# zhang-tao-whu/DVIS_Plus

Hardware: AMD Instinct MI355X
Metric: frames/sec DVIS++ R50 offline, 720p T=30 synthetic (higher is better)
Workload: dtype f32 (storage, accumulation, results; the segmenter's dense layers - R50 convolutions from 128 channels on, pixel-decoder projections and FPN output convolution, the deformable encoder's projections and FFN, the decoder's key / value projections - multiply each fp32 operand as two f16 terms on the f1

## Files before the change

### dvis_plus_amd/backbone.py

```python
import torch
import torch.nn.functional as F
from torch import nn

from . import derived, functions as Fn
from .registry import BACKBONE_REGISTRY, ShapeSpec


class FrozenBatchNorm2d(nn.Module):
    def __init__(self, num_features, eps=1e-5):
        super().__init__()
        self.num_features, self.eps = num_features, eps
        self.register_buffer("weight", torch.ones(num_features))
        self.register_buffer("bias", torch.zeros(num_features))
        self.register_buffer("running_mean", torch.zeros(num_features))
        self.register_buffer("running_var", torch.ones(num_features) - eps)

    def scale_shift(self):
        scale = self.weight * (self.running_var + self.eps).rsqrt()
        return scale, self.bias - self.running_mean * scale

    def forward(self, x):
        scale, shift = self.scale_shift()
        return x * scale.reshape(1, -1, 1, 1) + shift.reshape(1, -1, 1, 1)

# ... 151 lines not shown
        return {k: ShapeSpec(channels=self._out_channels[k], stride=2 ** int(k[3:]))
                for k in self._out_features}

    @staticmethod
    def _chain_blocks(stage):
        blocks = []
        for b in stage:
            convs = [b.conv1, b.conv2, b.conv3] + ([b.shortcut] if b.shortcut is not None else [])
            if any(c.stride != (1, 1) or c.dilation != (1, 1) or c.groups != 1 for c in convs) or b.conv2.padding != (1, 1) \
                    or any(c.padding != (0, 0) for c in (b.conv1, b.conv3)):
                return None
            (w1, b1), (w2, b2), (w3, b3) = b.conv1.folded(), b.conv2.folded(), b.conv3.folded()
            ws, bs = b.shortcut.folded() if b.shortcut is not None else (None, None)
            if any(key_is_channels_last(w) for w in (w1, w2, w3) + ((ws,) if ws is not None else ())):
                return None
            blocks.append(dict(w1=w1, b1=b1, w2=w2, b2=b2, w3=w3, b3=b3, ws=ws, bs=bs))
        return blocks

    def _forward_live(self, x):
        out = {}
        x = F.max_pool2d(F.relu(self.stem.conv1.live(x)), kernel_size=3, stride=2, padding=1)
        for name in self.stage_names:
            for b in getattr(self, name):
                y = F.relu(b.conv2.live(F.relu(b.conv1.live(x))))
                x = F.relu(b.conv3.live(y) + (x if b.shortcut is None else b.shortcut.live(x)))
            if name in self._out_features:
                out[name] = x
        return out

    @Fn.fp32_island
    def forward(self, x):
        if torch.is_grad_enabled() and any(p.requires_grad for p in self.parameters()):
            return self._forward_live(Fn.f32(x))
        out = {}
        x = self.stem(Fn.f32(x))
        for name in self.stage_names:
            stage = getattr(self, name)
            blocks = self._chain_blocks(stage) if name == "res2" and x.is_cuda and not torch.is_grad_enabled() else None
            if blocks is not None and Fn.bneck_stage_x3_ok(x, blocks):
                x = Fn.bneck_stage_x3(x, blocks)
            else:
                x = stage(x)
            if name in self._out_features:
                out[name] = x
        return out


def build_resnet50():
    return ResNet((3, 4, 6, 3))


@BACKBONE_REGISTRY.register()
def build_resnet_backbone(cfg, input_shape=None):
    r = cfg.MODEL.get("RESNETS", {}) if hasattr(cfg.MODEL, "get") else getattr(cfg.MODEL, "RESNETS", {})
    get = (lambda k, d: r.get(k, d)) if hasattr(r, "get") else (lambda k, d: getattr(r, k, d))
    if int(get("DEPTH", 50)) != 50 or bool(get("STRIDE_IN_1X1", False)) or get("NORM", "FrozenBN") != "FrozenBN":
        raise NotImplementedError("dvis_plus_amd serves ResNet-50 with FrozenBN and STRIDE_IN_1X1 False "
                                  "(the reference's R50 configs); use detectron2's builder for other ResNets")
    return ResNet((3, 4, 6, 3), tuple(get("OUT_FEATURES", ["res2", "res3", "res4", "res5"])))
```

### dvis_plus_amd/functions.py

```python
import collections
import ctypes
import math
import os
import threading

import torch
from torch.autograd import Function
from torch.autograd.function import once_differentiable

from . import cpu_ops, derived, native
from .cpu_ops import ms_deform_attn_core_pytorch


def _torch_path(op, x, why):
    if os.environ.get("DVIS_STRICT", "1") != "0" and x.is_cuda and not torch.is_grad_enabled():
        raise RuntimeError(f"DVIS_STRICT: {op} would run its torch formulation on a GPU tensor ({why}; shape "
                           f"{tuple(x.shape)}, dtype {x.dtype}, contiguous {x.is_contiguous()})")


class no_autocast:

    def __enter__(self):
        import contextlib
        self._stack = contextlib.ExitStack()
# ... 2377 lines not shown
                native.dev_ptr(out, "out"), N, C, K, H, W, 1 if relu else 0, native.stream_ptr(x.device))
        native.check(rc, "dvis_conv3x3s2")
        return out
    y = torch.nn.functional.conv2d(x, weight, None, 2, 1)
    if bias is None and not relu:
        return y
    return bias_act_(y, None if bias is None else bias.detach(), None, relu)


def conv7x7s2_stem(x, weight, bias=None, relu=False, own=None):
    N, C, H, W = x.shape
    K = weight.shape[0]
    ok = x.is_cuda and x.dtype == torch.float32 and weight.dtype == torch.float32 and tuple(weight.shape) == (64, 3, 7, 7) \
        and not (torch.is_grad_enabled() and (x.requires_grad or weight.requires_grad)) \
        and bool(native.lib().dvis_conv7x7s2_supported(C, K, H, W))
    if own and not ok:
        raise RuntimeError(f"conv7x7s2_stem(own=True): C={C} K={K} H={H} W={W} is not served (dvis_conv7x7s2_supported)")
    if ok and (own or (own is None and WINOGRAD_DEFAULT and S2_DEFAULT)):
        uf = _fp32_pack(weight, "conv7x7s2", 10240, native.lib().dvis_conv7x7s2_pack, "dvis_conv7x7s2_pack")
        x = x if x.is_contiguous() else x.contiguous()
        out = torch.empty((N, 64, H // 2, W // 2), dtype=torch.float32, device=x.device)
        with torch.cuda.device(x.device):
            rc = native.lib().dvis_conv7x7s2(native.dev_ptr(x, "x"), native.dev_ptr(uf, "uf"),
                                             None if bias is None else native.dev_ptr(bias.detach(), "bias"),
                                             native.dev_ptr(out, "out"), N, H, W, 1 if relu else 0, native.stream_ptr(x.device))
        native.check(rc, "dvis_conv7x7s2")
        return out
    y = torch.nn.functional.conv2d(x, weight, None, 2, 3)
    if bias is None and not relu:
        return y
    return bias_act_(y, None if bias is None else bias.detach(), None, relu)


def conv3x3_bias_act(x, weight, bias=None, relu=False, winograd=None):
    if winograd is None and weight.shape[1] >= 128 and conv3x3_x3_ok(x, weight, 1):
        return conv3x3_x3(x, weight, bias, None, relu, 1)
    use = WINOGRAD_DEFAULT if winograd is None else winograd
    if use and x.is_cuda and x.dim() == 4 and x.dtype == torch.float32 and weight.dtype == torch.float32 \
            and tuple(weight.shape[2:]) == (3, 3) and not (torch.is_grad_enabled() and (x.requires_grad or weight.requires_grad)):
        N, C, H, W = x.shape
        K = weight.shape[0]
        served = weight.shape[1] == C and native.lib().dvis_conv3x3_winograd_supported(C, K, H, W)
        if winograd and not served:
            raise RuntimeError(f"conv3x3_bias_act(winograd=True): shape C={C} K={K} H={H} W={W} is not served "
                               "(dvis_conv3x3_winograd_supported)")
        if served:
            x = x if x.is_contiguous() else x.contiguous()
            uf = _winograd_weights(weight)
            out = torch.empty((N, K, H, W), dtype=torch.float32, device=x.device)
            with torch.cuda.device(x.device):
                rc = native.lib().dvis_conv3x3_winograd(
                    native.dev_ptr(x, "x"), native.dev_ptr(uf, "uf"),
                    None if bias is None else native.dev_ptr(bias.detach(), "bias"), native.dev_ptr(out, "out"), N, C, K, H, W,
                    1 if relu else 0, native.stream_ptr(x.device))
            native.check(rc, "dvis_conv3x3_winograd")
            return out
    y = torch.nn.functional.conv2d(x, weight, None, 1, 1)
    if bias is None and not relu:
        return y
    return bias_act_(y, None if bias is None else bias.detach(), None, relu)


def bias_act_(x, bias=None, res=None, relu=True):
    N, C, H, W = x.shape
    if not (x.is_cuda and x.dtype == torch.float32 and x.is_contiguous()
            and (res is None or (res.is_contiguous() and res.shape == x.shape and res.dtype == torch.float32))
# ... 700 lines not shown
```

### dvis_plus_amd/meta_architecture.py

```python
import os

import numpy as np
import torch
from torch import nn

from . import d2
from . import functions as Fn
from . import native
from . import postprocess as PP
from .clip_shard import ClipShard, EmulatedShard
from .d2 import configurable
from .registry import META_ARCH_REGISTRY, SEM_SEG_HEADS_REGISTRY


def _get(node, key, default):
    if hasattr(node, "get"):
        return node.get(key, default)
    return getattr(node, key, default)


@SEM_SEG_HEADS_REGISTRY.register()
class MaskFormerHead(nn.Module):

    @configurable
# ... 36 lines not shown

@SEM_SEG_HEADS_REGISTRY.register()
class FCCLIPHead(MaskFormerHead):

    @configurable
    def __init__(self, input_shape=None, *, num_classes, pixel_decoder, loss_weight=1.0, ignore_value=-1, transformer_predictor,
                 transformer_in_feature):
        super().__init__(input_shape, num_classes=num_classes, pixel_decoder=pixel_decoder, loss_weight=loss_weight,
                         ignore_value=ignore_value, transformer_predictor=transformer_predictor,
                         transformer_in_feature=transformer_in_feature)

    @classmethod
    def from_config(cls, cfg, input_shape):
        ret = MaskFormerHead.from_config.__func__(cls, cfg, input_shape)
        del ret["return_transformer_feature"]
        return ret

    @Fn.fp32_island
    def forward(self, features, mask=None):
        mask_features, _, multi_scale_features = self.pixel_decoder.forward_features(features)
        return self.predictor(multi_scale_features, mask_features, mask, text_classifier=features["text_classifier"],
                              num_templates=features["num_templates"])

    def layers(self, features, mask=None):
        return self.forward(features, mask)


def segmenter_frames_per_call(n, H, W, requested=0):
    chunk = min(requested or max(1, n), max(1, n))
    if 0 < chunk < n:
        calls = (n + chunk - 1) // chunk
        chunk = (n + calls - 1) // calls
    return max(1, chunk)


class _VideoBase(nn.Module):

    @configurable
    def __init__(self, *, backbone, sem_seg_head, num_queries, object_mask_threshold=0.8, overlap_threshold=0.8,
                 n_things=0, size_divisibility=32, pixel_mean=(123.675, 116.280, 103.530),
                 pixel_std=(58.395, 57.120, 57.375), tracker=None, refiner=None, task="vis", max_num=20,
                 window_size=3, segmenter_chunk=0, metadata=None, criterion=None,
                 sem_seg_postprocess_before_inference=True, num_frames=1, window_inference=True, max_iter_num=0,
                 use_cl=False, reference_outputs=False):
        super().__init__()
        self.backbone, self.sem_seg_head, self.tracker, self.refiner = backbone, sem_seg_head, tracker, refiner
        self.num_queries = num_queries
        self.object_mask_threshold, self.overlap_threshold = object_mask_threshold, overlap_threshold
        self.metadata = metadata
        ids = d2.thing_ids_from_metadata(metadata, video=True)
        self.thing_ids = frozenset(range(int(n_things))) if ids is None else ids
        self.num_frames, self.window_inference = num_frames, window_inference
        self.criterion, self.max_iter_num, self.use_cl, self.iter = criterion, max_iter_num, use_cl, 0
        self.size_divisibility = size_divisibility
        self.register_buffer("pixel_mean", torch.tensor(pixel_mean, dtype=torch.float32).view(-1, 1, 1), False)
        self.register_buffer("pixel_std", torch.tensor(pixel_std, dtype=torch.float32).view(-1, 1, 1), False)
        assert task in ("vis", "vss", "vps")
        self.task, self.max_num = task, max_num
        self.reference_outputs = bool(reference_outputs)
        self.window_size = window_size
        self.segmenter_chunk = segmenter_chunk
        self.keep = False
        self._clip_shard = None
        self.pipeline_rounds = int(os.environ.get("DVIS_PIPELINE_ROUNDS", "1"))
        self._tracker_stream = None
        self.owner_rounds = os.environ.get("DVIS_OWNER_ROUNDS", "1") != "0"
# ... 43 lines not shown
                                       noise_mode=_get(trk, "NOISE_MODE", "none"),
                                       noise_ratio=_get(trk, "NOISE_RATIO", 0.5), mask_dim=mf.HIDDEN_DIM,
                                       class_num=cfg.MODEL.SEM_SEG_HEAD.NUM_CLASSES), hidden

    @staticmethod
    def _new_tracker_stream():
        return torch.cuda.Stream()

    @property
    def clip_shard(self):
        if isinstance(self._clip_shard, EmulatedShard):
            return self._clip_shard
        world = torch.distributed.get_world_size() if torch.distributed.is_initialized() else 1
        if self._clip_shard is None or self._clip_shard.world != world:
            self._clip_shard = ClipShard()
        return self._clip_shard

    def preprocess(self, frames):
        x = frames if torch.is_tensor(frames) else torch.stack([f.to(self.device) for f in frames])
        H, W = x.shape[-2:]
        d = self.size_divisibility
        Hp, Wp = ((H + d - 1) // d * d, (W + d - 1) // d * d) if d > 1 else (H, W)
        x = x.to(self.device)
        if x.is_cuda and x.dim() == 4 and not torch.is_grad_enabled():
            exact = x.dtype in (torch.int8, torch.int16, torch.float16, torch.bfloat16, torch.bool)
            x = (x.to(torch.float32) if exact else x).contiguous()
        if Fn.normalize_pad_ok(x, self.pixel_mean):
            return Fn.normalize_pad(x, self.pixel_mean, self.pixel_std, Hp, Wp), (H, W)
        x = (x.to(torch.float32) - self.pixel_mean) / self.pixel_std
        if (Hp, Wp) != (H, W):
            x = torch.nn.functional.pad(x, (0, Wp - W, 0, Hp - H))
        return x, (H, W)

    def prepare_targets(self, batched_inputs, images):
        Hp, Wp = images.shape[-2:]
        out = []
        for video in batched_inputs:
            frames = video["instances"]
            masks = torch.zeros((len(frames[0].gt_ids), len(frames), Hp, Wp), dtype=torch.bool, device=self.device)
            ids, classes = [], []
            for f, inst in enumerate(frames):
                m = getattr(inst.gt_masks, "tensor", inst.gt_masks).to(self.device)
                masks[:, f, :m.shape[-2], :m.shape[-1]] = m.bool()
                ids.append(inst.gt_ids.to(self.device)[:, None])
                classes.append(inst.gt_classes.to(self.device)[:, None])
            ids = torch.cat(ids, dim=1)
            classes = torch.cat(classes, dim=1).max(dim=1)[0]
            valid = (ids != -1).any(dim=-1)
            out.append({"labels": classes[valid], "ids": ids[valid], "masks": masks[valid].float()})
        return out

    def encode(self, images):
        chunk = segmenter_frames_per_call(len(images), images.shape[-2], images.shape[-1], self.segmenter_chunk)
        ms, mf = [], []
        for s in range(0, len(images), chunk):
            with Fn.x3_stage("backbone"):
                feats = self.backbone(images[s:s + chunk])
            f, _, m = self.sem_seg_head.pixel_decoder.forward_features(feats)
            mf.append(f)
            ms.append(m)
        if len(mf) == 1:
            return ms[0], mf[0]
        return [torch.cat(level, 0) for level in zip(*ms)], torch.cat(mf, 0)

    def decode(self, multi_scale, mask_features):
        if len(mask_features) == 0:
            pred = self.sem_seg_head.predictor
            C2, Q = self.tracker.decoder_norm.weight.shape[0], self.num_queries
            z = lambda *shape: mask_features.new_zeros(shape)
            return z(0, Q, C2), z(0, Q, C2), z(0, Q, pred.class_embed.out_features)
        out = self.sem_seg_head.predictor(multi_scale, mask_features, None)
        return (out["pred_embds"][0].permute(1, 2, 0), out["pred_embds_without_norm"][0].permute(1, 2, 0),
                out["pred_logits"][0])

    def segment(self, images):
        ms, mf = self.encode(images)
        return (*self.decode(ms, mf), mf)

    def _segmenter_graph_ok(self, images):
        limit = int(os.environ.get("DVIS_SEGMENTER_GRAPH", "8"))
        ok = bool(images.is_cuda and 0 < len(images) <= limit and not torch.is_grad_enabled() and self.debug_stages is None
                  and getattr(self.sem_seg_head.predictor, "debug_masks", None) is None)
        if ok and self._seg_graph is None:
            from .graphs import GraphRunner
            self._seg_graph = GraphRunner(lambda im: tuple(self.segment(im)), max_entries=4)
        return ok

    def _guard_snapshot(self):
        return Fn.x3_range_snapshot(self.device) if not getattr(self, "_x3_off", False) else None

# ... 117 lines not shown

        def run():
            with self._x3_scope(), Fn.x3_stage("backbone"):
                features = self.backbone(images)
            self._guard_verify(self._guard_snapshot())
            return features

        def again():
            with torch.no_grad():
                for b, v in saved:
                    b.copy_(v)
            return run()
        try:
            return run()
        except Fn.X3RangeError as e:
            return self._x3_rerun(e, again)

    @staticmethod
    def frame_decoder_loss_reshape(outputs, targets):
        def one(d):
            return {"pred_masks": d["pred_masks"].permute(0, 2, 1, 3, 4).flatten(0, 1).unsqueeze(2),
                    "pred_logits": d["pred_logits"].flatten(0, 1)}
        out = {**outputs, **one(outputs)}
        if "aux_outputs" in outputs:
            out["aux_outputs"] = [one(a) for a in outputs["aux_outputs"]]
        return out, _VideoBase._per_frame_targets(targets)

    @Fn.fp32_island
    def _forward_eval(self, batched_inputs):
        assert len(batched_inputs) == 1
        from . import functions as Fn
        from .tracker import match_chain
        video = batched_inputs[0]
        images, img_size = self.preprocess(video["image"])
        pred = self.sem_seg_head.predictor
        with self._x3_scope():
            ms, mask_features = self.encode(images)
            dec, logits, _ = pred._final_heads(pred._run_layers(ms, mask_features), mask_features, False)
        try:
            self._guard_verify(self._guard_snapshot())
        except Fn.X3RangeError as e:
            return self._x3_rerun(e, lambda: self._forward_eval(batched_inputs))
        T, Q, _ = dec.shape
        idx = torch.arange(Q, device=dec.device).unsqueeze(0).repeat(T, 1)
        if T > 1:
            align = self._alignment_embeds(pred, dec)
            nrm = align / align.norm(dim=-1, keepdim=True)
            cost = 1 - torch.bmm(nrm[1:], nrm[:-1].transpose(1, 2))
            idx[1:] = torch.from_numpy(match_chain(cost)).to(dec.device)
        ar = torch.arange(T, device=dec.device)[:, None]
        cls = logits[ar, idx].mean(0)
        K = self.sem_seg_head.num_classes
        scores, labels, slot = PP.vis_select(cls, K, self.TOPK)
        emb = pred.mask_embed(dec[ar, idx[:, slot]])
        masks = Fn.mask_logits(emb.contiguous(), mask_features).permute(1, 0, 2, 3)
        out_hw = (video.get("height", img_size[0]), video.get("width", img_size[1]))
        masks = PP.resize2_gt0(masks, images.shape[-2:], img_size, out_hw)
        out = {"image_size": tuple(out_hw), "pred_scores": scores.tolist(), "pred_labels": labels.tolist(),
               "pred_masks": [m for m in masks], "pred_ids": slot.tolist(), "aligned_indices": idx}
        return PP.to_reference_format(out) if self.reference_outputs else out


@META_ARCH_REGISTRY.register()
class CTMinVIS(MinVIS):

    @configurable
    def __init__(self, *, image_matcher=None, cl_plugin=None, **kwargs):
# ... 205 lines not shown
                                                   self.classes_references_memory))
        return self._weighted(losses)

    @staticmethod
    def frame_decoder_loss_reshape(outputs, targets, image_outputs=None):
        def one(d):
            b, q, t, h, w = d["pred_masks"].shape
            return {"pred_masks": d["pred_masks"].reshape(b, q, 1, t * h, w), "pred_logits": d["pred_logits"][:, 0]}
        out = one(outputs)
        out["pred_embds"] = outputs["pred_embds"]
        out["aux_outputs"] = [one(a) for a in outputs.get("aux_outputs", ())]
        if image_outputs is not None:
            b, q, t, h, w = image_outputs["pred_masks"].shape
            image_outputs = {"pred_masks": image_outputs["pred_masks"].reshape(b, q, 1, t * h, w),
                             "pred_logits": image_outputs["pred_logits"].mean(dim=1)}
        flat = []
        for t_ in targets:
            g, t, h, w = t_["masks"].shape
            flat.append({**t_, "masks": t_["masks"].reshape(g, 1, t * h, w)})
        return image_outputs, out, flat

    @torch.no_grad()
    def _segment_phase(self, video, shift=0):
        return self._segment_round([video], shift)[0]

    @torch.no_grad()
    def _segment_round(self, videos, shift=0, rotate=True):
        metas, batches = [], []
        for j, video in enumerate(videos):
            frames = video["image"]
            T = len(frames)
            sh = shift + j if rotate else shift
            lo, hi = self.clip_shard.local_range(T, sh)
            images, img_size = self.preprocess(frames[lo:hi] if hi > lo else frames[:1])
            metas.append(dict(video=video, T=T, lo=lo, hi=hi, shift=sh, img_size=img_size,
                              padded=tuple(images.shape[-2:])))
            batches.append(images if hi > lo else images[:0])
        mask_dim = self.sem_seg_head.predictor.mask_embed.layers[-1].out_features
        merged = len(videos) > 1 and len({m["padded"] for m in metas}) == 1 and sum(len(b) for b in batches) > 0 \
            and (self.clip_shard.world > 1 or self.clip_shard.force or "DVIS_ROUND_CLIPS" in os.environ)

        def run(images):
            if len(images):
                return self.segment(images)
            mf = images.new_zeros((0, mask_dim, images.shape[-2] // 4, images.shape[-1] // 4))
            return (*self.decode(None, mf), mf)
        with self._x3_scope():
            if merged:
                outs = run(torch.cat(batches, 0))
                sizes = [len(b) for b in batches]
                parts = [o.split(sizes, 0) for o in outs]
                per_clip = [tuple(p[j] for p in parts) for j in range(len(videos))]
            else:
                per_clip = [run(b) for b in batches]
        guard = self._guard_snapshot()
        for m, (e, e_nn, lg, mf) in zip(metas, per_clip):
            m.update(embds=e, embds_nn=e_nn, logits=lg, mf=mf, guard=guard)
            if self.debug_stages is not None:
                self.debug_stages.update(mask_features=mf)
        return metas

    @property
    def _resume(self):
        return bool(self.keep) and not self.window_inference

    def _track_core(self, embds, embds_nn):
        to_bctq = lambda z: z.permute(2, 0, 1).unsqueeze(0)
        embds, embds_nn = embds.contiguous(), embds_nn.contiguous()
        track = self.tracker(to_bctq(embds), None, resume=self._resume, frame_embeds_no_norm=to_bctq(embds_nn),
                             need_masks=False)
        ref = self.refiner(track["pred_embds"], to_bctq(embds_nn), None, need_masks=False)
        cls, aux = PP.mean_logits(ref["pred_logits"], track["pred_logits"])
        if self.debug_stages is not None:
            self.debug_stages.update(frame_embds=to_bctq(embds), frame_embds_no_norm=to_bctq(embds_nn),
                                     instance_embds=track["pred_embds"], online_logits=track["pred_logits"],
                                     refiner_embds=ref["pred_embds"], refiner_logits=ref["pred_logits"],
                                     refiner_mask_embed=ref["mask_embed"])
        return ref["mask_embed"], cls, aux

    def _finish_phase(self, st, mask_embed, cls, aux):
        video, lo, hi = st["video"], st["lo"], st["hi"]
        emb_local = mask_embed[:, lo:hi]
# ... 165 lines not shown
        return self._forward_eval(batched_inputs)

    @torch.no_grad()
    @Fn.fp32_island
    def _forward_eval(self, batched_inputs):
        assert len(batched_inputs) == 1 and not self.training
        video = batched_inputs[0]
        if self.pipeline_rounds <= 1:
            try:
                out = self._track_phase(self._segment_phase(video))
            except Fn.X3RangeError as e:
                out = self._x3_rerun(e, lambda: self._track_phase(self._segment_phase(video)))
            return PP.to_reference_format(out) if self.reference_outputs else out
        self.keep = bool(video.get("keep", False))
        frames = video["image"]
        T = len(frames)
        shard = self.clip_shard
        plan, k = shard.round_plan(T, self.pipeline_rounds)
        to_bctq = lambda z: z.permute(2, 0, 1).unsqueeze(0)
        overlap = len(plan) > 1 and self.device.type == "cuda"
        main = torch.cuda.current_stream() if overlap else None
        if overlap and self._tracker_stream is None:
            self._tracker_stream = self._new_tracker_stream()

        local_ids = [i for (_, _, lo, hi) in plan for i in range(lo, hi)]
        contiguous = local_ids == list(range(local_ids[0], local_ids[0] + len(local_ids))) if local_ids else True
        if not local_ids:
            mine = frames[:0] if torch.is_tensor(frames) else []
        elif contiguous:
            mine = frames[local_ids[0]:local_ids[0] + len(local_ids)]
        else:
            mine = frames[torch.as_tensor(local_ids, device=frames.device)] if torch.is_tensor(frames) \
                else [frames[i] for i in local_ids]
        images, img_size = self.preprocess(mine if local_ids else frames[:1])
        if not local_ids:
            images = images[:0]
            pred = self.sem_seg_head.predictor
            multi_scale = None
            mask_features = images.new_zeros((0, pred.mask_embed.layers[-1].out_features, images.shape[-2] // 4,
                                              images.shape[-1] // 4))
        else:
            multi_scale, mask_features = self.encode(images)
        padded = images.shape[-2:]
        offsets, o = [], 0
        for (_, _, lo, hi) in plan:
            offsets.append((o, o + hi - lo))
            o += hi - lo

        def run_segmenter(c):
            start, end, lo, hi = plan[c]
            a, b = offsets[c]
            whole = a == 0 and b == len(local_ids)
            ms = None if multi_scale is None else (multi_scale if whole else _slice_maps(multi_scale, a, b))
            e, e_nn, lg = self.decode(ms, mask_features[a:b])
            (e, e_nn, lg), work = shard.all_gather_frames([e, e_nn, lg], end - start, per=k, async_op=True)
            done = torch.cuda.Event() if overlap else None
            if overlap:
                done.record(main)
            return dict(embds=e, embds_nn=e_nn, logits=lg, work=work, done=done)

        def run_tracker(c, seg):
            if seg["work"] is not None:
                seg["work"].wait()
            return self.tracker(to_bctq(seg["embds"]), None, resume=self._resume or c > 0,
                                frame_embeds_no_norm=to_bctq(seg["embds_nn"]), need_masks=False)

        segs, tracks = [run_segmenter(0)], []
# ... 282 lines not shown
```

### dvis_plus_amd/native.py

```python
import ctypes
import os

import torch

_HERE = os.path.dirname(os.path.abspath(__file__))
LIB_PATH = os.environ.get("DVIS_HIP_LIB") or os.path.join(_HERE, "lib", "libdvis_hip.so")

F32, F64, F16, BF16 = 0, 1, 2, 3
_DTYPE = {torch.float32: F32, torch.float64: F64, torch.float16: F16, torch.bfloat16: BF16}

_c = ctypes
_i, _i64, _p, _f = _c.c_int, _c.c_int64, _c.c_void_p, _c.c_float

SIGNATURES = {
    "dvis_last_error": (_c.c_char_p, []),
    "dvis_version": (_i, []),
    "dvis_msda_forward": (_i, [_i, _p, _p, _p, _p, _p, _i, _i, _i, _i, _i, _i, _i, _p, _p]),
    "dvis_msda_backward": (_i, [_i, _p, _p, _p, _p, _p, _p, _i, _i, _i, _i, _i, _i, _i, _p, _p, _p, _p]),
    "dvis_msda_backward_det_ws_bytes": (_i64, [_i, _i, _i, _i]),
    "dvis_msda_backward_det": (_i, [_p, _p, _p, _p, _p, _p, _i, _i, _i, _i, _i, _i, _i, _p, _p, _p, _p, _p]),
    "dvis_msda_fused_backward_ws_bytes": (_i64, [_i, _i, _i, _i]),
    "dvis_msda_fused_backward": (_i, [_p, _p, _p, _p, _i, _p, _i64, _p, _i64, _p, _i, _i, _i, _i, _i, _i, _i, _p, _p, _p, _p, _p]),
    "dvis_msda_fused_forward": (_i, [_p, _p, _p, _p, _i, _p, _i64, _p, _i64, _i, _i, _i, _i, _i, _i, _i, _p, _p, _p]),
    "dvis_msda_fused_forward_h": (_i, [_i, _p, _p, _p, _p, _i, _p, _i64, _p, _i64, _i, _i, _i, _i, _i, _i, _i, _p, _p, _p]),
    "dvis_nchw_to_tokens": (_i, [_p, _p, _i64, _i, _i64, _i64, _i64, _p]),
    "dvis_tokens_to_nchw": (_i, [_p, _p, _i64, _i, _i64, _i64, _i64, _p]),
    "dvis_normalize_pad": (_i, [_p, _i, _p, _i64, _i, _i, _i, _i, _i, _p, _p, _p]),
    "dvis_nchw_to_tokens_affine": (_i, [_p, _p, _p, _p, _p, _p, _i64, _i, _i64, _i64, _i64, _p]),
    "dvis_mask_logits": (_i, [_p, _p, _i, _i, _i, _i64, _p, _p]),
    "dvis_mask_logits_backward_ws_bytes": (_i64, [_i, _i, _i, _i64]),
    "dvis_mask_logits_backward": (_i, [_p, _p, _i, _i, _i, _i64, _p, _p, _p, _p]),
    "dvis_attn_mask": (_i, [_p, _p, _i, _i, _i, _i, _i, _i, _i, _p, _p, _p]),
    "dvis_center_pool3": (_i, [_p, _i64, _i, _i, _p, _p, _p, _p]),
    "dvis_attn_mask_pooled": (_i, [_p, _p, _i, _i, _i, _i, _i, _p, _p, _p]),
    "dvis_mask_gemm_plan": (_i, [_i, _i, _i, _i, _i, _i, _i, _i, _i, _i, _p, _i]),
    "dvis_attention_ws_bytes": (_i64, [_i, _i, _i, _i]),
    "dvis_attention_ws_bytes_k": (_i64, [_i, _i, _i, _i, _i]),
    "dvis_attention_plan": (_i, [_i, _i, _i, _i, _i, _i64, _i64, _i, _p]),
    "dvis_attention_forward": (_i, [_p, _p, _p, _p, _p, _p, _p, _p, _p, _p, _i, _i, _i, _i, _i, _f, _p, _p]),
    "dvis_attention_forward_k": (_i, [_p, _p, _p, _p, _p, _p, _p, _p, _p, _p, _i, _i, _i, _i, _i, _f, _p, _p, _i]),
    "dvis_attention_backward": (_i, [_p, _p, _p, _p, _p, _p, _p, _p, _p, _p, _p, _i, _i, _i, _i, _i, _f, _p]),
    "dvis_attention_backward_threads": (_i, [_i]),
    "dvis_masked_attention_backward_ws_bytes": (_i64, [_i, _i, _i, _i]),
    "dvis_masked_attention_backward": (_i, [_p, _p, _p, _p, _p, _p, _p, _p, _p, _p, _p, _p, _p, _i, _i, _i, _i, _i, _f, _p, _p]),
    "dvis_masked_attention_backward_plan": (_i, [_i, _i, _i, _p]),
    "dvis_add_layernorm": (_i, [_p, _p, _i64, _p, _p, _p, _i64, _i, _f, _p]),
    "dvis_add_layernorm_pos": (_i, [_p, _p, _i64, _p, _p, _p, _p, _i64, _p, _i64, _i, _f, _p]),
    "dvis_bias_act": (_i, [_p, _p, _p, _i64, _i, _i64, _i, _p]),
    "dvis_conv3x3_winograd_supported": (_i, [_i, _i, _i, _i]),
    "dvis_conv3x3_winograd_pack": (_i, [_p, _p, _i, _i, _p]),
    "dvis_conv3x3_winograd": (_i, [_p, _p, _p, _p, _i, _i, _i, _i, _i, _i, _p]),
    "dvis_conv3x3s2_supported": (_i, [_i, _i, _i, _i]),
    "dvis_conv3x3s2_pack": (_i, [_p, _p, _i, _i, _p]),
    "dvis_conv3x3s2": (_i, [_p, _p, _p, _p, _i, _i, _i, _i, _i, _i, _p]),
    "dvis_conv7x7s2_supported": (_i, [_i, _i, _i, _i]),
    "dvis_conv7x7s2_pack": (_i, [_p, _p, _p]),
    "dvis_conv7x7s2": (_i, [_p, _p, _p, _p, _i, _i, _i, _i, _p]),
    "dvis_conv1x1_mfma_supported": (_i, [_i, _i, _i64]),
    "dvis_conv1x1_mfma_pack": (_i, [_p, _p, _i, _i, _p]),
    "dvis_conv1x1_mfma": (_i, [_p, _p, _p, _p, _p, _i, _i, _i, _i64, _i, _p]),
    "dvis_conv1x1s2_mfma": (_i, [_p, _p, _p, _p, _p, _i, _i, _i, _i, _i, _i, _p]),
    "dvis_conv1x1_supported": (_i, [_i, _i, _i64]),
    "dvis_conv1x1_bias_act": (_i, [_p, _p, _p, _p, _p, _i, _i, _i, _i64, _i, _p]),
    "dvis_bias_relu_maxpool": (_i, [_p, _p, _p, _i64, _i, _i, _i, _p]),
    "dvis_group_norm_affine": (_i, [_p, _p, _p, _p, _p, _i64, _i, _i, _i64, _f, _p]),
    "dvis_scale_shift_act": (_i, [_p, _p, _p, _i64, _i64, _i, _p]),
    "dvis_group_norm_finalize": (_i, [_p, _p, _p, _p, _p, _i64, _i, _i, _i64, _f, _p]),
    "dvis_upsample_add_affine": (_i, [_p, _p, _p, _p, _p, _i64, _i, _i, _i, _i, _p]),
    "dvis_upsample_add": (_i, [_p, _p, _p, _i64, _i, _i, _i, _i, _p]),
    "dvis_dwconv3x3_tokens": (_i, [_p, _p, _i64, _i, _i, _i, _i, _p, _p, _i, _p]),
    "dvis_dwconv3x3_tokens_backward_ws_bytes": (_i64, [_i, _i, _i, _i]),
    "dvis_dwconv3x3_tokens_backward": (_i, [_p, _p, _p, _p, _i, _i64, _i, _i, _i, _i, _p, _p, _p, _p, _p]),
    "dvis_adapter_res2": (_i, [_p, _p, _p, _p, _p, _p, _i, _i, _i, _i, _p]),
    "dvis_vps_argmax": (_i, [_p, _i64, _i64, _p, _i, _i, _i, _i, _i, _i, _i, _i, _i, _i, _p, _p, _p, _p]),
    "dvis_vss_argmax": (_i, [_p, _i64, _i64, _p, _i, _i, _i, _i, _i, _i, _i, _i, _i, _i, _i, _i, _p, _p]),
    "dvis_resize2_gt0": (_i, [_p, _i64, _i64, _i, _i, _i, _i, _i, _i, _i, _i, _i, _i, _p, _p]),
    "dvis_resize2": (_i, [_p, _i64, _i64, _i, _i, _i, _i, _i, _i, _i, _i, _i, _i, _i, _p, _p]),
    "dvis_lsap_solve": (_i, [_p, _i, _i, _p]),
    "dvis_match_chain": (_i, [_p, _i, _i, _p]),
    "dvis_gemm_nt": (_i, [_p, _i64, _i64, _p, _i64, _i64, _p, _p, _i64, _i64, _p, _i64, _i64, _i, _i, _i, _i, _i, _i, _p]),
    "dvis_gemm_nt_bb": (_i, [_p, _i64, _i64, _p, _i64, _i64, _p, _i64, _p, _i64, _i64, _p, _i64, _i64, _i, _i, _i, _i, _i, _i,
                             _p]),
    "dvis_gemm_ln": (_i, [_p, _i64, _p, _i64, _p, _p, _f, _p, _p, _f, _p, _i64, _p, _i64, _p, _p, _i64, _p, _i64, _i, _i, _i,
                          _i, _i, _p]),
    "dvis_gemm_ln_supported": (_i, [_i, _i, _i, _i]),
    "dvis_gemm_ln_num_configs": (_i, []),
    "dvis_gemm_ln_pick_config": (_i, [_i, _i, _i]),
    "dvis_x3_packed_bytes": (_i64, [_i, _i]),
    "dvis_x3_set_reserve": (_i, [_i]),
    "dvis_x3_set_range_flag": (_i, [_p]),
# ... 124 lines not shown
```

### include/dvis_hip.h

```cpp
#ifndef DVIS_HIP_H
#define DVIS_HIP_H

#include <stdint.h>

#ifdef __cplusplus
extern "C" {
#endif

enum { DVIS_F32 = 0, DVIS_F64 = 1, DVIS_F16 = 2, DVIS_BF16 = 3 };

enum {
  DVIS_OK = 0,
  DVIS_E_ARG = -1,
  DVIS_E_LAUNCH = -2,
  DVIS_E_UNSUPPORTED = -3
};

const char *dvis_last_error(void);
int dvis_version(void);

int dvis_msda_forward(int dtype, const void *value, const int64_t *shapes, const int64_t *level_start,
                      const void *loc, const void *w, int N, int S, int M, int D, int L, int Lq, int P,
                      void *out, void *stream);

// ... 74 lines not shown
int dvis_add_layernorm(const float *x, const float *res, int64_t res_row_stride, const float *gamma, const float *beta,
                       float *out, int64_t rows, int C, float eps, void *stream);

int dvis_add_layernorm_pos(const float *x, const float *res, int64_t res_row_stride, const float *gamma, const float *beta,
                           float *out, const float *pos, int64_t pos_rows, float *out_pos, int64_t rows, int C, float eps,
                           void *stream);

int dvis_upsample_add(const float *lateral, const float *top, float *out, int64_t planes, int H, int W, int h, int w,
                      void *stream);

int dvis_nchw_to_tokens(const float *x, float *out, int64_t N, int C, int64_t HW, int64_t S, int64_t row0, void *stream);

int dvis_tokens_to_nchw(const float *tok, float *out, int64_t N, int C, int64_t HW, int64_t S, int64_t row0, void *stream);
int dvis_normalize_pad(const void *in, int is_u8, float *out, int64_t planes, int C, int H, int W, int Hp, int Wp, const float *mean,
                       const float *stdv, void *stream);
int dvis_nchw_to_tokens_affine(const float *x, const float *scale, const float *shift, const float *pos, float *out,
                               float *out_pos, int64_t N, int C, int64_t HW, int64_t S, int64_t row0, void *stream);

int dvis_conv1x1_supported(int K, int M, int64_t HW);
int dvis_conv1x1_mfma_supported(int C, int K, int64_t HW);
int dvis_conv1x1_mfma_pack(const float *w, float *uf, int K, int C, void *stream);
int dvis_conv1x1_mfma(const float *x, const float *uf, const float *bias, const float *res, float *y, int N, int C, int K, int64_t HW,
                      int relu, void *stream);
int dvis_conv1x1s2_mfma(const float *x, const float *uf, const float *bias, const float *res, float *y, int N, int C, int K, int H, int W,
                        int relu, void *stream);
int dvis_conv1x1_bias_act(const float *x, const float *w, const float *bias, const float *res, float *out,
                          int N, int K, int M, int64_t HW, int relu, void *stream);

int dvis_conv3x3_winograd_supported(int C, int K, int H, int W);
int dvis_conv3x3s2_supported(int C, int K, int H, int W);
int dvis_conv7x7s2_supported(int C, int K, int H, int W);
int dvis_conv7x7s2_pack(const float *w, float *uf, void *stream);
int dvis_conv7x7s2(const float *x, const float *uf, const float *bias, float *y, int N, int H, int W, int relu, void *stream);
int dvis_conv3x3s2_pack(const float *w, float *uf, int K, int C, void *stream);
int dvis_conv3x3s2(const float *x, const float *uf, const float *bias, float *y, int N, int C, int K, int H, int W, int relu,
                   void *stream);
int dvis_conv3x3_winograd_pack(const float *w, float *uf, int K, int C, void *stream);
int dvis_conv3x3_winograd(const float *x, const float *uf, const float *bias, float *y, int N, int C, int K, int H, int W,
                          int relu, void *stream);

int dvis_bias_act(float *x, const float *bias, const float *res, int64_t planes, int C, int64_t HW, int relu,
                  void *stream);

int dvis_bias_relu_maxpool(const float *x, const float *bias, float *out, int64_t planes, int C, int H, int W,
                           void *stream);

int dvis_group_norm_affine(const float *x, const float *gamma, const float *beta, float *scale, float *shift, int64_t N,
                           int C, int G, int64_t HW, float eps, void *stream);
int dvis_scale_shift_act(float *x, const float *scale, const float *shift, int64_t planes, int64_t HW, int relu,
                         void *stream);
int dvis_group_norm_finalize(const double *part, const float *gamma, const float *beta, float *scale, float *shift, int64_t N, int C,
                             int G, int64_t HW, float eps, void *stream);
int dvis_upsample_add_affine(const float *lateral, const float *lat_scale, const float *lat_shift, const float *top,
                             float *out, int64_t planes, int H, int W, int h, int w, void *stream);

int dvis_dwconv3x3_tokens(const float *x, float *out, int64_t batch_stride, int B, int h, int w, int C, const float *weight,
                          const float *bias, int gelu, void *stream);

int64_t dvis_dwconv3x3_tokens_backward_ws_bytes(int B, int h, int w, int C);
int dvis_dwconv3x3_tokens_backward(const float *x, const float *grad_out, const float *weight, const float *bias, int gelu,
                                   int64_t batch_stride, int B, int h, int w, int C, float *grad_x, float *grad_weight, float *grad_bias,
                                   void *ws, void *stream);

int dvis_adapter_res2(const float *g, const float *c1, const float *x1, const float *scale, const float *shift, float *out, int B, int C,
                      int h8, int w8, void *stream);

// ... 181 lines not shown
```

Before: 428.5.

## Fuse uint8 normalize, pad, 7x7 stem conv, bias-ReLU and maxpool into one kernel

Adds a HIP kernel that reads raw uint8 frames, normalizes them through a per-channel lookup table in LDS and zero-pads them on the fly. It then runs the 7x7 stride-2 stem convolution with fp32 MFMA, applies bias and ReLU, and does the 3x3 stride-2 max pool, writing only the pooled output. Video preprocessing is rerouted to carry a lazy _RawFrames wrapper so the backbone can use this path and skip materializing the normalized fp32 image and the full-resolution stem output. The cost is a new batch-wrapper abstraction with fallback paths. Stem tiles are recomputed per pooled tile with halo overlap.

```diff
diff --git a/dvis_plus_amd/backbone.py b/dvis_plus_amd/backbone.py
--- a/dvis_plus_amd/backbone.py
+++ b/dvis_plus_amd/backbone.py
@@ -207,8 +207,23 @@
     def forward(self, x):
         if torch.is_grad_enabled() and any(p.requires_grad for p in self.parameters()):
             return self._forward_live(Fn.f32(x))
+        return self._stages(self.stem(Fn.f32(x)))
+
+    def frames_ok(self, frames, mean, std, Hp, Wp):
+        c = self.stem.conv1
+        if not (c.kernel_size == (7, 7) and c.stride == (2, 2) and c.padding == (3, 3) and c.dilation == (1, 1) and c.groups == 1
+                and c.in_channels == 3 and c.out_channels == 64) or torch.is_grad_enabled():
+            return False
+        w, _ = c.folded()
+        return not key_is_channels_last(w) and Fn.stem_u8_pool_ok(frames, mean, std, Hp, Wp, w)
+
+    @Fn.fp32_island
+    def forward_frames(self, frames, mean, std, Hp, Wp):
+        w, b = self.stem.conv1.folded()
+        return self._stages(Fn.stem_u8_pool(frames, mean, std, Hp, Wp, w, b))
+
+    def _stages(self, x):
         out = {}
-        x = self.stem(Fn.f32(x))
         for name in self.stage_names:
             stage = getattr(self, name)
             blocks = self._chain_blocks(stage) if name == "res2" and x.is_cuda and not torch.is_grad_enabled() else None
diff --git a/dvis_plus_amd/csrc/stem_u8.hip b/dvis_plus_amd/csrc/stem_u8.hip
--- /dev/null
+++ b/dvis_plus_amd/csrc/stem_u8.hip
@@ -0,0 +1,190 @@
+#include "dvis_common.h"
+
+namespace {
+
+constexpr int kPH = 4, kPW = 16;
+constexpr int kSR = 2 * kPH + 1, kSC = 2 * kPW + 1;
+constexpr int kSPix = kSR * kSC, kTiles = (kSPix + 15) / 16;
+constexpr int kIR = 2 * kSR + 5, kIC = 2 * kSC + 5;
+constexpr int kPitch = 73, kPlane = kIR * kPitch;
+constexpr int kQ = (kIC + 3) / 4, kTasks = 3 * kIR * kQ;
+constexpr int kThreads = 256, kFill = (kTasks + kThreads - 1) / kThreads;
+constexpr int kSP = 300;
+constexpr int kLdsPatch = 0, kLdsStem = (3 * kPlane + 3) & ~3, kLdsTab = kLdsStem;
+constexpr int kLdsFloats = kLdsStem + 16 * kSP;
+static_assert(768 <= 16 * kSP, "the table fits the stem tile's place");
+constexpr unsigned kOOB = 0x80000000u;
+static_assert(kIC + 1 <= kPitch && 4 * kQ <= kPitch, "patch pitch");
+static_assert((2 * kPlane + 6 * kPitch + 6) * 4 < 65536, "row offsets are packed as 16-bit byte offsets");
+static_assert(kSPix <= kSP, "stem tile pitch");
+
+struct StemU8Args {
+  const unsigned char *frames;
+  const float *uf, *shift, *mean, *stdv;
+  float *out;
+  int H, W, OH, OW, PH, PW;
+};
+
+__device__ __forceinline__ unsigned row_off(int r) {
+  if (r >= 147) return 0u;
+  const int c = r / 49, q = r - 49 * c, ky = q / 7, kx = q - 7 * ky;
+  return (unsigned)(c * kPlane + ky * kPitch + kx) * 4u;
+}
+
+__global__ __launch_bounds__(kThreads, 4) void stem_u8_pool_kernel(const StemU8Args a) {
+  extern __shared__ float lds[];
+  const int tid = threadIdx.x, lane = tid & 63;
+  const int wv = __builtin_amdgcn_readfirstlane(tid >> 6);
+  const int j = lane & 15, g = lane >> 4;
+  const int px0 = blockIdx.x * kPW, py0 = blockIdx.y * kPH, n = blockIdx.z;
+  const int ix0 = 4 * px0 - 5, iy0 = 4 * py0 - 5;
+
+  const unsigned img = 3u * (unsigned)a.H * (unsigned)a.W;
+  const uintptr_t fb = (uintptr_t)a.frames + (uintptr_t)n * img;
+  const unsigned delta = (unsigned)(fb & 3);
+  const __amdgpu_buffer_rsrc_t rf = dvis_make_rsrc_uniform((const void *)(fb - delta), (img + delta + 3u) & ~3u);
+  const __amdgpu_buffer_rsrc_t ru = dvis_make_rsrc_uniform(a.uf, (unsigned)(4 * 2 * 64 * 20 * 4));
+
+  unsigned word[kFill];
+#pragma unroll
+  for (int t = 0; t < kFill; ++t) {
+    const int id = tid + kThreads * t;
+    const int cr = id / kQ, q = id - cr * kQ, c = cr / kIR, r = cr - c * kIR;
+    const int iy = iy0 + r, ix = ix0 + 4 * q;
+    const bool need = id < kTasks && iy >= 0 && iy < a.H && ix + 3 >= 0 && ix < a.W;
+    const int rowbase = (int)delta + (c * a.H + iy) * a.W, rowal = rowbase & ~3;
+    const int a0 = rowbase + ix, al = a0 & ~3, sh = a0 & 3;
+    const bool l0 = need && al >= rowal && al < rowbase + a.W;
+    const bool l1 = need && sh != 0 && al + 4 >= rowal && al + 4 < rowbase + a.W;
+    const unsigned w0 = __builtin_amdgcn_raw_buffer_load_b32(rf, l0 ? (unsigned)al : kOOB, 0, 0);
+    const unsigned w1 = __builtin_amdgcn_raw_buffer_load_b32(rf, l1 ? (unsigned)(al + 4) : kOOB, 0, 0);
+    word[t] = __builtin_amdgcn_alignbyte(w1, w0, (unsigned)sh);
+  }
+
+  for (int i = tid; i < 768; i += kThreads) {
+    const int c = i >> 8;
+    lds[kLdsTab + i] = __fdiv_rn(__fsub_rn((float)(i & 255), a.mean[c]), a.stdv[c]);
+  }
+  __syncthreads();
+#pragma unroll
+  for (int t = 0; t < kFill; ++t) {
+    const int id = tid + kThreads * t;
+    if (id >= kTasks) break;
+    const int cr = id / kQ, q = id - cr * kQ, c = cr / kIR, r = cr - c * kIR;
+    const int iy = iy0 + r, ix = ix0 + 4 * q;
+    const bool rowok = iy >= 0 && iy < a.H;
+    float *pw = lds + kLdsPatch + c * kPlane + r * kPitch + 4 * q;
+#pragma unroll
+    for (int e = 0; e < 4; ++e) {
+      const unsigned u = (word[t] >> (8 * e)) & 255u;
+      const int x = ix + e;
+      pw[e] = (rowok && x >= 0 && x < a.W) ? lds[kLdsTab + c * 256 + (int)u] : 0.f;
+    }
+  }
+
+  unsigned offs[19];
+#pragma unroll
+  for (int s = 0; s < 19; ++s) offs[s] = row_off(4 * s + g) | (s < 18 ? row_off(4 * (19 + s) + g) << 16 : 0u);
+  __syncthreads();
+
+  const int tg = (wv + (int)blockIdx.x + (int)blockIdx.y) & 3;
+  const char *pb = reinterpret_cast<const char *>(lds + kLdsPatch);
+  float *stem = lds + kLdsStem;
+  dvis_f4 u0[5], u1[5];
+  auto load_weights = [&](int ps) {
+    const unsigned ubase = (unsigned)(ps * 2) * 5120u;
+#pragma unroll
+    for (int q = 0; q < 5; ++q) {
+      u0[q] = __builtin_bit_cast(dvis_f4, __builtin_amdgcn_raw_buffer_load_b128(ru, (unsigned)lane * 16u + 1024u * q, ubase, 0));
+      u1[q] = __builtin_bit_cast(dvis_f4,
+                                 __builtin_amdgcn_raw_buffer_load_b128(ru, (unsigned)lane * 16u + 1024u * q, ubase + 5120u, 0));
+    }
+  };
+  load_weights(0);
+  for (int ps = 0; ps < 4; ++ps) {
+    for (int t = tg; t < kTiles; t += 4) {
+      const int p = 16 * t + j, pc = min(p, kSPix - 1);
+      const int sr = pc / kSC, sc = pc - sr * kSC;
+      const char *bp = pb + (2 * sr * kPitch + 2 * sc) * 4;
+      dvis_f4 acc0 = {0.f, 0.f, 0.f, 0.f}, acc1 = {0.f, 0.f, 0.f, 0.f};
+      float b0[19], b1[18];
+#pragma unroll
+      for (int s = 0; s < 19; ++s) {
+        b0[s] = *reinterpret_cast<const float *>(bp + (offs[s] & 0xffffu));
+        if (s < 18) b1[s] = *reinterpret_cast<const float *>(bp + (offs[s] >> 16));
+      }
+      __builtin_amdgcn_sched_barrier(0);
+#pragma unroll
+      for (int s = 0; s < 19; ++s) {
+        acc0 = __builtin_amdgcn_mfma_f32_16x16x4f32(u0[s >> 2][s & 3], b0[s], acc0, 0, 0, 0);
+        if (s < 18) acc1 = __builtin_amdgcn_mfma_f32_16x16x4f32(u1[s >> 2][s & 3], b1[s], acc1, 0, 0, 0);
+      }
+      const int sy = 2 * py0 - 1 + sr, sx = 2 * px0 - 1 + sc;
+      const bool inmap = sy >= 0 && sy < a.OH && sx >= 0 && sx < a.OW;
+      if (p < kSPix) {
+        float *sw = stem + (4 * g) * kSP + p;
+#pragma unroll
+        for (int rr = 0; rr < 4; ++rr) sw[rr * kSP] = inmap ? acc0[rr] + acc1[rr] : -INFINITY;
+      }
+    }
+    if (ps < 3) load_weights(ps + 1);
+    __syncthreads();
+
+    {
+      const int ch = tid >> 4, py = (tid >> 2) & 3, xq = tid & 3;
+      const float *sp = stem + ch * kSP + (2 * py) * kSC + 8 * xq;
+      float m[9];
+#pragma unroll
+      for (int i = 0; i < 9; ++i) m[i] = -INFINITY;
+#pragma unroll
+      for (int dy = 0; dy < 3; ++dy)
+#pragma unroll
+        for (int i = 0; i < 9; ++i) m[i] = fmaxf(m[i], sp[dy * kSC + i]);
+      const float bb = a.shift[16 * ps + ch];
+      dvis_f4 o;
+      o[0] = fmaxf(fmaxf(fmaxf(m[0], m[1]), m[2]) + bb, 0.f);
+      o[1] = fmaxf(fmaxf(fmaxf(m[2], m[3]), m[4]) + bb, 0.f);
+      o[2] = fmaxf(fmaxf(fmaxf(m[4], m[5]), m[6]) + bb, 0.f);
+      o[3] = fmaxf(fmaxf(fmaxf(m[6], m[7]), m[8]) + bb, 0.f);
+      const int oy = py0 + py, ox = px0 + 4 * xq;
+      if (oy < a.PH && ox < a.PW)
+        *reinterpret_cast<dvis_f4 *>(a.out + (((size_t)n * 64 + 16 * ps + ch) * a.PH + oy) * (size_t)a.PW + ox) = o;
+    }
+    if (ps < 3) __syncthreads();
+  }
+}
+
+}
+
+DVIS_EXPORT int dvis_stem_u8_pool_supported(int H, int W, int Hp, int Wp) {
+  if (H <= 0 || W <= 0 || Hp < H || Wp < W || (Hp & 3) || (Wp & 15)) return 0;
+  if ((long long)(Hp / 2) * (Wp / 2) < 64 || 3ll * H * W + 4 >= (1ll << 31)) return 0;
+  if ((Hp / 4 + kPH - 1) / kPH > 65535) return 0;
+  return 1;
+}
+
+DVIS_EXPORT int dvis_stem_u8_pool(const void *frames_u8, int N, int H, int W, int Hp, int Wp, const float *mean, const float *stdv,
+                                  const float *uf, const float *shift, float *out, void *stream) {
+  DVIS_REQUIRE(N >= 0, "stem_u8_pool: bad batch");
+  if (N == 0) return DVIS_OK;
+  DVIS_REQUIRE(frames_u8 && mean && stdv && uf && shift && out, "stem_u8_pool: null pointer");
+  DVIS_REQUIRE(dvis_stem_u8_pool_supported(H, W, Hp, Wp),
+               "stem_u8_pool: unsupported size H=%d W=%d Hp=%d Wp=%d (dvis_stem_u8_pool_supported)", H, W, Hp, Wp);
+  DVIS_REQUIRE((((uintptr_t)uf | (uintptr_t)out) & 15) == 0, "stem_u8_pool: 16-byte aligned uf / out");
+  static DvisLdsOptIn opted;
+  const size_t lds_bytes = kLdsFloats * sizeof(float);
+  if (int rc = dvis_lds_opt_in((const void *)stem_u8_pool_kernel, lds_bytes, &opted, "dvis_stem_u8_pool")) return rc;
+  StemU8Args a;
+  a.uf = uf, a.shift = shift, a.mean = mean, a.stdv = stdv;
+  a.H = H, a.W = W, a.OH = Hp / 2, a.OW = Wp / 2, a.PH = Hp / 4, a.PW = Wp / 4;
+  const size_t img = (size_t)3 * H * W, oimg = (size_t)64 * a.PH * a.PW;
+  for (int n0 = 0; n0 < N; n0 += 32768) {
+    const int nn = N - n0 < 32768 ? N - n0 : 32768;
+    a.frames = (const unsigned char *)frames_u8 + (size_t)n0 * img;
+    a.out = out + (size_t)n0 * oimg;
+    const dim3 grid((unsigned)((a.PW + kPW - 1) / kPW), (unsigned)((a.PH + kPH - 1) / kPH), (unsigned)nn);
+    hipLaunchKernelGGL(stem_u8_pool_kernel, grid, dim3(kThreads), lds_bytes, (hipStream_t)stream, a);
+    if (int rc = dvis_check_launch("dvis_stem_u8_pool")) return rc;
+  }
+  return DVIS_OK;
+}
diff --git a/dvis_plus_amd/functions.py b/dvis_plus_amd/functions.py
--- a/dvis_plus_amd/functions.py
+++ b/dvis_plus_amd/functions.py
@@ -2433,6 +2433,38 @@
     return bias_act_(y, None if bias is None else bias.detach(), None, relu)
 
 
+STEM_U8 = os.environ.get("DVIS_STEM_U8", "1") != "0"
+
+
+def stem_u8_pool_ok(frames, mean, std, Hp, Wp, weight=None):
+    if not (STEM_U8 and torch.is_tensor(frames) and frames.is_cuda and frames.dim() == 4 and frames.dtype == torch.uint8
+            and frames.shape[1] == 3 and frames.is_contiguous() and not torch.is_grad_enabled()
+            and mean.numel() == 3 and std.numel() == 3 and mean.dtype == std.dtype == torch.float32
+            and mean.device == std.device == frames.device):
+        return False
+    if weight is not None and not (weight.dtype == torch.float32 and tuple(weight.shape) == (64, 3, 7, 7)
+                                   and weight.device == frames.device):
+        return False
+    H, W = frames.shape[-2:]
+    return bool(native.lib().dvis_stem_u8_pool_supported(H, W, Hp, Wp))
+
+
+def stem_u8_pool(frames, mean, std, Hp, Wp, weight, shift):
+    if not stem_u8_pool_ok(frames, mean, std, Hp, Wp, weight):
+        return bias_relu_maxpool(conv7x7s2_stem(normalize_pad(frames, mean, std, Hp, Wp), weight), shift)
+    N, _, H, W = frames.shape
+    uf = _fp32_pack(weight, "conv7x7s2", 10240, native.lib().dvis_conv7x7s2_pack, "dvis_conv7x7s2_pack")
+    out = torch.empty((N, 64, Hp // 4, Wp // 4), dtype=torch.float32, device=frames.device)
+    with torch.cuda.device(frames.device):
+        rc = native.lib().dvis_stem_u8_pool(
+            native.dev_ptr(frames, "frames"), N, H, W, Hp, Wp, native.dev_ptr(mean.detach().reshape(-1), "pixel_mean"),
+            native.dev_ptr(std.detach().reshape(-1), "pixel_std"), native.dev_ptr(uf, "uf"),
+            native.dev_ptr(shift.detach().float().contiguous(), "shift"), native.dev_ptr(out, "out"),
+            native.stream_ptr(frames.device))
+    native.check(rc, "dvis_stem_u8_pool")
+    return out
+
+
 def conv3x3_bias_act(x, weight, bias=None, relu=False, winograd=None):
     if winograd is None and weight.shape[1] >= 128 and conv3x3_x3_ok(x, weight, 1):
         return conv3x3_x3(x, weight, bias, None, relu, 1)
diff --git a/dvis_plus_amd/meta_architecture.py b/dvis_plus_amd/meta_architecture.py
--- a/dvis_plus_amd/meta_architecture.py
+++ b/dvis_plus_amd/meta_architecture.py
@@ -92,6 +92,38 @@
         calls = (n + chunk - 1) // chunk
         chunk = (n + calls - 1) // calls
     return max(1, chunk)
+
+
+class _RawFrames:
+
+    def __init__(self, frames, mean, std, Hp, Wp):
+        self.frames, self.mean, self.std = frames, mean, std
+        self.shape = torch.Size((frames.shape[0], frames.shape[1], Hp, Wp))
+        self.device, self.is_cuda, self.dtype = frames.device, frames.is_cuda, torch.float32
+
+    def __len__(self):
+        return self.shape[0]
+
+    def __getitem__(self, idx):
+        if not isinstance(idx, slice):
+            raise TypeError("_RawFrames takes frame slices")
+        return _RawFrames(self.frames[idx], self.mean, self.std, *self.shape[-2:])
+
+    def args(self):
+        return self.frames, self.mean, self.std, self.shape[-2], self.shape[-1]
+
+    def new_zeros(self, shape):
+        return torch.zeros(tuple(shape), dtype=torch.float32, device=self.device)
+
+    def tensor(self):
+        return Fn.normalize_pad(*self.args())
+
+    @staticmethod
+    def cat(batches):
+        raw = [b for b in batches if isinstance(b, _RawFrames)]
+        if len(raw) == len(batches) and len({tuple(b.frames.shape[1:]) for b in raw}) == 1:
+            return _RawFrames(torch.cat([b.frames for b in raw], 0), raw[0].mean, raw[0].std, *raw[0].shape[-2:])
+        return torch.cat([b.tensor() if isinstance(b, _RawFrames) else b for b in batches], 0)
 
 
 class _VideoBase(nn.Module):
@@ -201,6 +233,24 @@
             x = torch.nn.functional.pad(x, (0, Wp - W, 0, Hp - H))
         return x, (H, W)
 
+    def frames_to_backbone(self, frames):
+        bb = self.backbone
+        if hasattr(bb, "forward_frames") and not torch.is_grad_enabled():
+            x = frames if torch.is_tensor(frames) else torch.stack([f.to(self.device) for f in frames])
+            x = x.to(self.device)
+            if x.dim() == 4 and x.dtype == torch.uint8:
+                x = x.contiguous()
+                H, W = x.shape[-2:]
+                d = self.size_divisibility
+                Hp, Wp = ((H + d - 1) // d * d, (W + d - 1) // d * d) if d > 1 else (H, W)
+                if bb.frames_ok(x, self.pixel_mean, self.pixel_std, Hp, Wp):
+                    return _RawFrames(x, self.pixel_mean, self.pixel_std, Hp, Wp), (H, W)
+            frames = x
+        return self.preprocess(frames)
+
+    def backbone_features(self, images):
+        return self.backbone.forward_frames(*images.args()) if isinstance(images, _RawFrames) else self.backbone(images)
+
     def prepare_targets(self, batched_inputs, images):
         Hp, Wp = images.shape[-2:]
         out = []
@@ -224,7 +274,7 @@
         ms, mf = [], []
         for s in range(0, len(images), chunk):
             with Fn.x3_stage("backbone"):
-                feats = self.backbone(images[s:s + chunk])
+                feats = self.backbone_features(images[s:s + chunk])
             f, _, m = self.sem_seg_head.pixel_decoder.forward_features(feats)
             mf.append(f)
             ms.append(m)
@@ -408,7 +458,7 @@
         from . import functions as Fn
         from .tracker import match_chain
         video = batched_inputs[0]
-        images, img_size = self.preprocess(video["image"])
+        images, img_size = self.frames_to_backbone(video["image"])
         pred = self.sem_seg_head.predictor
         with self._x3_scope():
             ms, mask_features = self.encode(images)
@@ -680,7 +730,7 @@
             T = len(frames)
             sh = shift + j if rotate else shift
             lo, hi = self.clip_shard.local_range(T, sh)
-            images, img_size = self.preprocess(frames[lo:hi] if hi > lo else frames[:1])
+            images, img_size = self.frames_to_backbone(frames[lo:hi] if hi > lo else frames[:1])
             metas.append(dict(video=video, T=T, lo=lo, hi=hi, shift=sh, img_size=img_size,
                               padded=tuple(images.shape[-2:])))
             batches.append(images if hi > lo else images[:0])
@@ -695,7 +745,7 @@
             return (*self.decode(None, mf), mf)
         with self._x3_scope():
             if merged:
-                outs = run(torch.cat(batches, 0))
+                outs = run(_RawFrames.cat(batches))
                 sizes = [len(b) for b in batches]
                 parts = [o.split(sizes, 0) for o in outs]
                 per_clip = [tuple(p[j] for p in parts) for j in range(len(videos))]
@@ -927,7 +977,7 @@
         else:
             mine = frames[torch.as_tensor(local_ids, device=frames.device)] if torch.is_tensor(frames) \
                 else [frames[i] for i in local_ids]
-        images, img_size = self.preprocess(mine if local_ids else frames[:1])
+        images, img_size = self.frames_to_backbone(mine if local_ids else frames[:1])
         if not local_ids:
             images = images[:0]
             pred = self.sem_seg_head.predictor
diff --git a/dvis_plus_amd/native.py b/dvis_plus_amd/native.py
--- a/dvis_plus_amd/native.py
+++ b/dvis_plus_amd/native.py
@@ -56,6 +56,8 @@
     "dvis_conv7x7s2_supported": (_i, [_i, _i, _i, _i]),
     "dvis_conv7x7s2_pack": (_i, [_p, _p, _p]),
     "dvis_conv7x7s2": (_i, [_p, _p, _p, _p, _i, _i, _i, _i, _p]),
+    "dvis_stem_u8_pool_supported": (_i, [_i, _i, _i, _i]),
+    "dvis_stem_u8_pool": (_i, [_p, _i, _i, _i, _i, _i, _p, _p, _p, _p, _p, _p]),
     "dvis_conv1x1_mfma_supported": (_i, [_i, _i, _i64]),
     "dvis_conv1x1_mfma_pack": (_i, [_p, _p, _i, _i, _p]),
     "dvis_conv1x1_mfma": (_i, [_p, _p, _p, _p, _p, _i, _i, _i, _i64, _i, _p]),
diff --git a/include/dvis_hip.h b/include/dvis_hip.h
--- a/include/dvis_hip.h
+++ b/include/dvis_hip.h
@@ -130,6 +130,9 @@
 int dvis_conv7x7s2_supported(int C, int K, int H, int W);
 int dvis_conv7x7s2_pack(const float *w, float *uf, void *stream);
 int dvis_conv7x7s2(const float *x, const float *uf, const float *bias, float *y, int N, int H, int W, int relu, void *stream);
+int dvis_stem_u8_pool_supported(int H, int W, int Hp, int Wp);
+int dvis_stem_u8_pool(const void *frames_u8, int N, int H, int W, int Hp, int Wp, const float *mean, const float *stdv,
+                      const float *uf, const float *shift, float *out, void *stream);
 int dvis_conv3x3s2_pack(const float *w, float *uf, int K, int C, void *stream);
 int dvis_conv3x3s2(const float *x, const float *uf, const float *bias, float *y, int N, int C, int K, int H, int W, int relu,
                    void *stream);
```

New measurement: 428.4, median of 2. No clear change (-0.0%).
